# limix/CellRegMap

Hardware: AMD Instinct MI355X
Metric: variant-tests/sec (interaction test) (higher is better)
Workload: dtype f64

## Files before the change

cellregmap_amd/csrc/api_core.hip:

```cpp
#include <dlfcn.h>

#include <algorithm>
#include <atomic>
#include <cstdarg>
#include <mutex>

#include <map>

#include "crm_internal.h"
#include "eigh.h"

namespace crm {

static thread_local std::string g_error;

void set_error(const char* fmt, ...) {
    char buf[1024];
    va_list ap;
    va_start(ap, fmt);
    vsnprintf(buf, sizeof buf, fmt, ap);
    va_end(ap);
    g_error = buf;
}

// ... 216 lines not shown
    }
}

int crm_ctx_synchronize(crm_ctx* c) {
    return crm::guarded_on("crm_ctx_synchronize", c, [&]() -> int {
    if (!c) return CRM_ERR_ARG;
    CRM_HIP(hipSetDevice(c->device));
    CRM_HIP(hipStreamSynchronize(c->stream));
    return CRM_OK;
    });
}

int crm_set_block_variants(crm_ctx* c, int variants) {
    return crm::guarded_on("crm_set_block_variants", c, [&]() -> int {
    if (!c || variants < 0) return CRM_ERR_ARG;
    c->block_variants = variants == 0 ? 0 : (int)round_up(variants, 128);
    return CRM_OK;
    });
}

int crm_set_null_fit_polish(crm_ctx* c, int on) {
    return crm::guarded_on("crm_set_null_fit_polish", c, [&]() -> int {
    if (!c) return CRM_ERR_ARG;
    c->polish = on != 0;
    return CRM_OK;
    });
}

int crm_set_progress_callback(crm_ctx* c, void (*callback)(long, long, void*), void* user) {
    return crm::guarded_on("crm_set_progress_callback", c, [&]() -> int {
    if (!c) return CRM_ERR_ARG;
    if (callback) c->progress[std::this_thread::get_id()] = crm_ctx::Progress{callback, user};
    else c->progress.erase(std::this_thread::get_id());
    return CRM_OK;
    });
}

int crm_set_fast_rotation(crm_ctx* c, int on) {
    return crm::guarded_on("crm_set_fast_rotation", c, [&]() -> int {
    if (!c) return CRM_ERR_ARG;
    c->fast_T = on != 0;
    return CRM_OK;
    });
}

extern "C++" {
namespace crm {
namespace {
struct FormSlot { const char* name; int value; bool set; };
FormSlot g_forms[] = {{"gram_staged", 0, false}, {"kr_no_tail", 0, false}, {"nullfit_per_wave", 0, false}, {"kin_fold", 0, false},
                      {"eigh_one_stage", 0, false}, {"nullfit_exact", 0, false}, {"donor_pairs", 0, false},
                      {"pairs_without_kinship_term", 0, false}, {"flat_kappa_milli", 0, false}, {"chase_abort", 0, false}, {"nullfit_one_per_wave", 0, false},
                      {"kin_diag", 0, false}, {"donor_pairs_rotate", 0, false}, {"rho0_positions", 0, false},
                      {"rotation_tails", 0, false}};
std::mutex g_forms_mu;
}
int form(const char* name, int otherwise) {
    std::lock_guard<std::mutex> lock(g_forms_mu);
    for (const FormSlot& f : g_forms)
        if (strcmp(f.name, name) == 0) return f.set ? f.value : otherwise;
    return otherwise;
}
}
}

int crm_test_set_form(const char* name, int value, int reset) {
    return crm::guarded("crm_test_set_form", [&]() -> int {
    if (!name) return CRM_ERR_ARG;
    std::lock_guard<std::mutex> lock(crm::g_forms_mu);
    for (crm::FormSlot& f : crm::g_forms)
        if (strcmp(f.name, name) == 0) {
            f.value = value;
            f.set = reset == 0;
            return CRM_OK;
        }
    crm::set_error("crm_test_set_form: no kernel form is called '%s'", name);
    return CRM_ERR_ARG;
    });
}

int crm_kernel_timer_reset(crm_ctx* c) {
    return crm::guarded_on("crm_kernel_timer_reset", c, [&]() -> int {
    if (!c) return CRM_ERR_ARG;
    CRM_HIP(hipSetDevice(c->device));
    CRM_HIP(hipStreamSynchronize(c->stream));
    c->timed_used = 0;
    c->kr_flops = 0.0;
    c->timing = true;
    return CRM_OK;
    });
}

int crm_kernel_timer_stop(crm_ctx* c) {
    return crm::guarded_on("crm_kernel_timer_stop", c, [&]() -> int {
    if (!c) return CRM_ERR_ARG;
    c->timing = false;
    return CRM_OK;
    });
}

int crm_kernel_timer_read(crm_ctx* c, double* kr_ms, long* kr_launches, double* kr_flops,
                          double* total_ms) {
    return crm::guarded_on("crm_kernel_timer_read", c, [&]() -> int {
    if (!c) return CRM_ERR_ARG;
    CRM_HIP(hipSetDevice(c->device));
    CRM_HIP(hipStreamSynchronize(c->stream));
    double ms = 0.0;
// ... 250 lines not shown
```

cellregmap_amd/csrc/assemble.hip:

```cpp
#include <type_traits>

#include "nullfit.h"

namespace crm {

namespace {

constexpr int CH = 64;
constexpr int SLD = 66;

typedef double v4d __attribute__((ext_vector_type(4)));

template <int NTL, int NG = 1>
__global__ __launch_bounds__(256) void gram_ext_kernel(AssembleArgs a, double* __restrict__ Gext, int KT) {
    constexpr int ROWS = 16 * NTL, NTILES = NTL * (NTL + 1) / 2, NLOC = (NTILES + NG - 1) / NG, MAXT = (NLOC + 3) / 4,
                  RPT = ROWS / 4;
    extern __shared__ double Ss[];
    __shared__ int tile_ij[NTILES];
    __shared__ const double* tail_ptr[ROWS];
    const int b = blockIdx.x;
    const NullFitOut fit = a.fit[b];
    const AssembleRho R = a.rho[fit.rho_index];
    const int r = R.r;
    const double ratio = fit.v0 / fit.v1;
// ... 469 lines not shown
    }
    double* ME = wsm;
    double* Cm = ME + KT * k1;
    double* Z = Cm + k1 * k1;
    const long pos = a.sorted_pos[b];
    for (int e = tid; e < KT * k1; e += 256) {
        const int u = e / k1, f = e - u * k1;
        double plain;
        if (u < k0) plain = pos >= 0 ? a.wb_E1X[(long)f * a.wb_ldE1X + pos * k0 + u] : 0.0;
        else if (u < k0 + c) plain = a.wb_E1yW[(long)f * a.wb_ldE1yW + 1 + (u - k0)];
        else if (u == k0 + c) plain = a.wb_E1g[(long)f * a.wb_ldE1g + b];
        else plain = a.wb_E1yW[(long)f * a.wb_ldE1yW];
        ME[e] = (u < k0 && pos < 0) ? 0.0 : (plain - G[(long)u * KW + KT + f]) * inv;
    }
    for (int e = tid; e < k1 * k1; e += 256) {
        const int i = e / k1, j = e - i * k1;
        Cm[e] = (i == j ? 1.0 : 0.0) + g * (a.wb_EE[e] - G[(long)(KT + i) * KW + KT + j]) * inv;
    }
    __syncthreads();
    for (int j = 0; j < k1; j++) {
        if (tid == 0) Cm[j * k1 + j] = sqrt(Cm[j * k1 + j]);
        __syncthreads();
        const double l = Cm[j * k1 + j];
        for (int i = j + 1 + tid; i < k1; i += 256) Cm[i * k1 + j] /= l;
        __syncthreads();
        for (int e = tid; e < (k1 - j - 1) * (k1 - j - 1); e += 256) {
            const int i = j + 1 + e / (k1 - j - 1), q = j + 1 + e % (k1 - j - 1);
            if (q <= i) Cm[i * k1 + q] -= Cm[i * k1 + j] * Cm[q * k1 + j];
        }
        __syncthreads();
    }
    for (int u = tid; u < KT; u += 256) {
        for (int i = 0; i < k1; i++) {
            double s = ME[u * k1 + i];
            for (int q = 0; q < i; q++) s -= Cm[i * k1 + q] * Z[q * KT + u];
            Z[i * KT + u] = s / Cm[i * k1 + i];
        }
        for (int i = k1 - 1; i >= 0; i--) {
            double s = Z[i * KT + u];
            for (int q = i + 1; q < k1; q++) s -= Cm[q * k1 + i] * Z[q * KT + u];
            Z[i * KT + u] = s / Cm[i * k1 + i];
        }
    }
    __syncthreads();
    const double scale = fit.v1 * g;
    for (int e = tid; e < KT * KT; e += 256) {
        const int u = e / KT, v = e - u * KT;
        double s = 0.0;
        for (int f = 0; f < k1; f++) s += ME[u * k1 + f] * Z[f * KT + v];
        out[e] = G[(long)u * KW + v] + scale * s;
    }
}

constexpr int PMAX = CRM_MAX_COV_XWIDE + 1;

__global__ __launch_bounds__(128) void finalize_kernel(AssembleArgs a, const double* __restrict__ Gext,
                                                        int KT, double* __restrict__ rows) {
    extern __shared__ double fsm[];
    __shared__ int ok_flag, keep_flag;
    __shared__ double rescale;
    const int Pd = a.c + 1;
    double* Lm = fsm;
    double* xky = Lm + Pd * Pd;
    double* uvec = xky + Pd;
    double* vv = uvec + a.k0;
    double* ww = vv + Pd;
    double* dkxm = rows ? rows + (size_t)blockIdx.x * 2 * a.k0 * Pd : ww + Pd;
    double* solm = dkxm + a.k0 * Pd;
#define L(i, j) Lm[(i) * Pd + (j)]
#define dkx(j, i) dkxm[(j) * Pd + (i)]
#define sol(j, i) solm[(j) * Pd + (i)]
    const int b = blockIdx.x;
    const NullFitOut fit = a.fit[b];
    const int k0 = a.k0, c = a.c;
    const int P = c + 1;
    const double v1 = fit.v1;
    const double inv = 1.0 / v1;
    const double* __restrict__ Ge = Gext + (long)b * KT * KT;
    const int tid = threadIdx.x;
    auto plain_xx = [&](int i, int j) -> double {
        if (i > j) { int t = i; i = j; j = t; }
        if (j < c) return a.WW[i * c + j];
        if (i < c) return a.gW[(long)b * a.ld_gW + i];
        return a.gg[b];
    };
    auto plain_xy = [&](int i) -> double { return i < c ? a.Wy[i] : a.gy[b]; };

    if (tid == 0) {
        bool ok = true;
        for (int i = 0; i < P; i++) {
            for (int j = 0; j <= i; j++)
                L(i, j) = (plain_xx(i, j) - Ge[(long)(k0 + i) * KT + (k0 + j)]) * inv;
            xky[i] = (plain_xy(i) - Ge[(long)(k0 + i) * KT + (k0 + c + 1)]) * inv;
        }
        bool keep = true;
        for (int j = 0; j < P && ok; j++) {
            double d = L(j, j);
            for (int k = 0; k < j; k++) d -= L(j, k) * L(j, k);
            if (!(d > 0.0)) {
                if (j == c) keep = false;
                else ok = false;
                break;
            }
            const double l = sqrt(d);
            L(j, j) = l;
            for (int i = j + 1; i < P; i++) {
                double s = L(i, j);
                for (int k = 0; k < j; k++) s -= L(i, k) * L(j, k);
                L(i, j) = s / l;
            }
// ... 58 lines not shown
                for (int i = 0; i < used; i++) r -= xky[i] * xky[i];
                const double df = (double)a.n - (double)(c + (fit.use_g ? 1 : 0));
                rescale = 1.0 / fmax(r / df, 1.4901161193847656e-08);
            }
            for (int i = P - 1; i >= 0; i--) {
                double s = xky[i];
                for (int k = i + 1; k < P; k++) s -= L(k, i) * xky[k];
                xky[i] = s / L(i, i);
            }
        }
        ok_flag = ok ? 1 : 0;
    }
    __syncthreads();
    const bool ok = ok_flag != 0;
    const bool keep_g = keep_flag != 0;
    for (int j = tid; j < k0; j += blockDim.x) {
        double row[PMAX];
        for (int i = 0; i < P; i++) {
            double plain;
            if (i < c) plain = a.Z1[(long)b * a.ldZ1 + (long)(1 + i) * k0 + j];
            else plain = a.Z2[(long)b * a.ldZ2 + j];
            double v = (plain - Ge[(long)j * KT + (k0 + i)]) * inv;
            if (i == c && !keep_g) v = 0.0;
            row[i] = v;
            dkx(j, i) = v;
        }
        for (int i = 0; i < P; i++) {
            double s = row[i];
            for (int k = 0; k < i; k++) s -= L(i, k) * row[k];
            row[i] = s / L(i, i);
        }
        for (int i = P - 1; i >= 0; i--) {
            double s = row[i];
            for (int k = i + 1; k < P; k++) s -= L(k, i) * row[k];
            row[i] = s / L(i, i);
        }
        for (int i = 0; i < P; i++) sol(j, i) = row[i];
        const double dky = (a.Z1[(long)b * a.ldZ1 + j] - Ge[(long)j * KT + (k0 + c + 1)]) * inv;
        double u = dky;
        for (int i = 0; i < P; i++) u -= dkx(j, i) * xky[i];
        uvec[j] = u * rescale;
    }
    __syncthreads();
    if (tid == 0) {
        double q = 0.0;
        for (int j = 0; j < k0; j++) q += uvec[j] * uvec[j];
        a.Q[b] = ok ? 0.5 * q : NAN;
    }
    double* __restrict__ F = a.F + (long)b * k0 * k0;
    for (int e = tid; e < k0 * k0; e += blockDim.x) {
        const int j = e / k0, jp = e - j * k0;
        const int lo = j < jp ? j : jp, hi = j < jp ? jp : j;
        const long pidx = (long)lo * k0 - (long)lo * (lo - 1) / 2 + (hi - lo);
        double v = (a.Z3[(long)b * a.ldZ3 + pidx] - Ge[(long)j * KT + jp]) * inv;
        for (int i = 0; i < P; i++) v -= dkx(j, i) * sol(jp, i);
        F[e] = ok ? 0.5 * v * rescale : NAN;
    }
}
#undef L
#undef dkx
#undef sol

}

size_t woodbury_lds_bytes(int KT, int k1) { return sizeof(double) * ((size_t)2 * KT * k1 + (size_t)k1 * k1); }

size_t assemble_rows_scratch_doubles(int variants, int k0, int c) {
    const size_t P = (size_t)c + 1;
    const size_t lds = sizeof(double) * (P * P + 3 * P + k0 + 2 * (size_t)k0 * P);
    return lds > 150 * 1024 ? (size_t)variants * 2 * k0 * P : 0;
}

int launch_assemble(hipStream_t st, const AssembleArgs& a, int variants, double* Gext, double* fin_rows,
                    long* dma_launches) {
    if (variants <= 0) return CRM_OK;
    const int KT0 = a.k0 + a.c + 2;
    const int KT = KT0 + (a.wb_k1 > 0 ? a.wb_k1 : 0);
    double* const Gfin = Gext;
    if (a.wb_k1 > 0) {
        if (KT > CRM_MAX_GRAM_ROWS || woodbury_lds_bytes(KT0, a.wb_k1) > 150 * 1024 || !a.wb_Gw) {
            set_error("assemble: unrelated-donor form with %d + %d rows outside its supported range", KT0, a.wb_k1);
            return CRM_ERR_INTERNAL;
        }
        Gext = a.wb_Gw;
    }
    const int P = a.c + 1;
    const size_t fin_small = sizeof(double) * ((size_t)P * P + 3 * P + a.k0);
    size_t fin_lds = fin_small + sizeof(double) * 2 * (size_t)a.k0 * P;
    const bool rows_global = fin_lds > 150 * 1024;
    if (rows_global) fin_lds = fin_small;
    if (a.k0 > CRM_MAX_K0 || a.c > CRM_MAX_COV_XWIDE || KT > CRM_MAX_GRAM_ROWS || (rows_global && !fin_rows)) {
        set_error("assemble: k0=%d, c=%d outside the supported range (k0 <= %d, c <= %d, k0 + c + 2 <= %d)", a.k0, a.c,
                  CRM_MAX_K0, CRM_MAX_COV_XWIDE, CRM_MAX_GRAM_ROWS);
        return CRM_ERR_UNSUPPORTED;
    }
    const int ts = (KT + 15) / 16;
    bool dma = ts <= 9 && a.ldA % 2 == 0 && (reinterpret_cast<uintptr_t>(a.A) & 15) == 0 && !form("gram_staged", 0);
    for (int i = 0; dma && i < CRM_MAX_RHO; i++) {
        const AssembleRho& R = a.rho[i];
        if (R.r <= 0 && !R.ty) continue;
        dma = R.ldW % 2 == 0 && R.ldT % 2 == 0 && ((reinterpret_cast<uintptr_t>(R.ty) | reinterpret_cast<uintptr_t>(R.tW) |
                                                    reinterpret_cast<uintptr_t>(R.T)) & 15) == 0;
    }
    if (a.wb_k1 > 0) dma = dma && a.wb_ldR % 2 == 0 && (reinterpret_cast<uintptr_t>(a.wb_R) & 15) == 0;
#define CRM_GRAM_DMA(KERNEL, LDS_DOUBLES, NTL)                                                                \
    do {                                                                                                      \
        const size_t lds = sizeof(double) * LDS_DOUBLES(NTL);                                                 \
        if (lds > 60 * 1024)                                                                                  \
            CRM_HIP(hipFuncSetAttribute(reinterpret_cast<const void*>(&KERNEL<NTL>),                          \
                                        hipFuncAttributeMaxDynamicSharedMemorySize, (int)lds));               \
        hipLaunchKernelGGL(KERNEL<NTL>, dim3(variants), dim3(256), lds, st, a, Gext, KT);                     \
    } while (0)
#define CRM_GRAM_DMA_WIDE(NTL) CRM_GRAM_DMA(gram_ext_dma_wide_kernel, gram_dma_wide_lds_doubles, NTL)
    if (dma) {
        if (ts <= 2) CRM_GRAM_DMA(gram_ext_dma_kernel, gram_dma_lds_doubles, 2);
        else if (ts <= 4) CRM_GRAM_DMA(gram_ext_dma_kernel, gram_dma_lds_doubles, 4);
        else if (ts == 5) CRM_GRAM_DMA_WIDE(5);
        else if (ts == 6) CRM_GRAM_DMA_WIDE(6);
        else if (ts == 7) CRM_GRAM_DMA_WIDE(7);
        else if (ts == 8) CRM_GRAM_DMA_WIDE(8);
        else CRM_GRAM_DMA_WIDE(9);
    }
#undef CRM_GRAM_DMA_WIDE
#undef CRM_GRAM_DMA
#define CRM_GRAM(NTL)                                                                                         \
    do {                                                                                                      \
        const size_t lds = sizeof(double) * 16 * NTL * SLD;                                                   \
        if (lds > 60 * 1024)                                                                                  \
            CRM_HIP(hipFuncSetAttribute(reinterpret_cast<const void*>(&gram_ext_kernel<NTL>),                 \
                                        hipFuncAttributeMaxDynamicSharedMemorySize, (int)lds));               \
        hipLaunchKernelGGL(gram_ext_kernel<NTL>, dim3(variants), dim3(256), lds, st, a, Gext, KT);            \
    } while (0)
#define CRM_GRAM_GROUPS(NTL, NG)                                                                              \
    do {                                                                                                      \
        const size_t lds = sizeof(double) * 16 * NTL * SLD;                                                   \
        CRM_HIP(hipFuncSetAttribute(reinterpret_cast<const void*>(&gram_ext_kernel<NTL, NG>),                 \
                                    hipFuncAttributeMaxDynamicSharedMemorySize, (int)lds));                   \
        hipLaunchKernelGGL((gram_ext_kernel<NTL, NG>), dim3(variants, NG), dim3(256), lds, st, a, Gext, KT);  \
    } while (0)
    if (dma) {
    } else if (ts <= 2) CRM_GRAM(2);
    else if (ts <= 4) CRM_GRAM(4);
    else if (ts <= 6) CRM_GRAM(6);
    else if (ts <= 7) CRM_GRAM(7);
    else if (ts <= 9) CRM_GRAM(9);
    else if (ts <= 12) CRM_GRAM_GROUPS(12, 2);
    else if (ts <= 15) CRM_GRAM_GROUPS(15, 4);
    else CRM_GRAM_GROUPS(18, 4);
#undef CRM_GRAM
#undef CRM_GRAM_GROUPS
    CRM_HIP(hipGetLastError());
    if (dma && dma_launches) ++*dma_launches;
    if (a.wb_k1 > 0) {
        const size_t lds = woodbury_lds_bytes(KT0, a.wb_k1);
        if (lds > 60 * 1024)
            CRM_HIP(hipFuncSetAttribute(reinterpret_cast<const void*>(&woodbury_kernel),
                                        hipFuncAttributeMaxDynamicSharedMemorySize, (int)lds));
        hipLaunchKernelGGL(woodbury_kernel, dim3(variants), dim3(256), lds, st, a, a.wb_Gw, KT0, Gfin);
        CRM_HIP(hipGetLastError());
    }
    if (fin_lds > 60 * 1024)
        CRM_HIP(hipFuncSetAttribute(reinterpret_cast<const void*>(&finalize_kernel),
                                    hipFuncAttributeMaxDynamicSharedMemorySize, (int)fin_lds));
    hipLaunchKernelGGL(finalize_kernel, dim3(variants), dim3(128), fin_lds, st, a, Gfin, KT0, rows_global ? fin_rows : nullptr);
    CRM_HIP(hipGetLastError());
    return CRM_OK;
}

}
```

cellregmap_amd/csrc/scan.hip:

```cpp
#include <algorithm>

#include "nullfit.h"
#include "objects.h"

using namespace crm;

namespace crm {

static int ctx_cus(const crm_ctx* ctx) {
    int cus = 256;
    if (hipDeviceGetAttribute(&cus, hipDeviceAttributeMultiprocessorCount, ctx->device) != hipSuccess || cus < 1) cus = 256;
    return cus;
}

constexpr double COLLINEAR_TAU = 1e-2;

__global__ void flat_probe_fit_kernel(const crm::NullFitOut* __restrict__ fit, int count, double sign,
                                      crm::NullFitOut* __restrict__ out) {
    const int b = blockIdx.x * blockDim.x + threadIdx.x;
    if (b >= count) return;
    crm::NullFitOut f = fit[b];
    const double tiny = 2.220446049250313e-16;
    const double d = fmin(fmax(f.delta, tiny), 1.0 - tiny);
    const double x = log(d) - log1p(-d);
// ... 11 lines not shown
    const int b = blockIdx.y;
    const int j = blockIdx.x * blockDim.x + threadIdx.x;
    if (b >= nb || j >= cols) return;
    const int ri = fit[b].rho_index;
    if (ri < 0) return;
    double* slab = T + ((size_t)ri * blk + b) * ldT;
    if (restore) slab[j] = rows[(size_t)b * ldT + j];
    else rows[(size_t)b * ldT + j] = slab[j];
}

constexpr double STOP_SHIFT_C = 2.5e-13;
constexpr double FLAT_KAPPA = 1.0;
constexpr double RHO_KAPPA = 1.0;
constexpr int FLAT_REC = 10;

struct ScanOut {
    double *pv, *rho1, *e2, *g2, *eps2, *Q, *lml, *delta, *scale, *lambda, *F;
    int* ifault = nullptr;
    double* liu = nullptr;
    int* flags = nullptr;
    double* bound_Q = nullptr;
    double* bound_p = nullptr;
    bool exact = false;
    double* logp = nullptr;
    int* status = nullptr;
};

static bool scan_slow_forms(const crm_gene* g0) {
    return g0->k0 + g0->c + 2 > 144 || g0->k0 > 128 || assemble_rows_scratch_doubles(1, g0->k0, g0->c) > 0;
}
static int scan_block_variants(const crm_ctx* ctx, const crm_gene* g0, long count) {
    long auto_blk = (long)(16.0 * (1ull << 30) / (sizeof(double) * (double)g0->k0 * (double)g0->bg->ldq)) / 128 * 128;
    auto_blk = std::max<long>(256, std::min<long>(auto_blk, CRM_MAX_AUTO_BLOCK));
    int BLK = (int)std::min<long>(ctx->block_variants > 0 ? ctx->block_variants : auto_blk, round_up(count, 128));
    if (g0->c > CRM_MAX_COV_WIDE) BLK = std::min(BLK, 512);
    if (scan_slow_forms(g0)) BLK = std::min(BLK, 512);
    return BLK;
}

enum class Route {
    collapsed,
    direct,
    kin_unfolded,
    kin_folded,
    unrelated,
};

constexpr int SLOT_ONE = 0, SLOT_RHO = 1, SLOT_KIN = 2 * CRM_MAX_RHO + 4;

struct ScanPlan {
    Route route = Route::direct;
    bool fastT = false, slow_forms = false, skip_pairs = true, cross = false;
    bool e1_pairs = false, e1_sym = false, donor_pairs = false, wb_rotate = false, pairs_unfolded = false;
    int ng = 1, BLK = 0, pair_cap = 0;
    long ldb = 0, ldp = 0, ldA = 0, ldAw = 0, ldT = 0, ldZ1 = 0, ldZ2 = 0, ldZ3 = 0, ld_ah = 0, ld_xg = 0, ldP = 0, ldPd = 0,
         pd_slab = 0, ldwb = 0, ld_gW = 0, th_slab = 0, s_rows = 0;
    size_t s_bytes = 0;
    int ks1 = 1, ks2 = 1, ks3 = 1, ks_h = 1, fold_split6 = 1, fold_split3 = 1, donor_pair_splits = 1;
    int npair = 0, KT = 0, KK = 0, kin_probs = 0;
    long kdim = 0, mp = 0, xrows = 0;
    bool collapsed() const { return route == Route::collapsed; }
    bool kin() const { return route == Route::kin_unfolded || route == Route::kin_folded || route == Route::unrelated; }
    bool folded() const { return route == Route::kin_folded || route == Route::unrelated; }
    bool wb() const { return route == Route::unrelated; }
    bool through_H() const { return fastT && (ng > 1 || kin()); }
    int z1_slot() const { return SLOT_KIN + kin_probs; }
};

static double largest_rank(const crm_background* bg) {
    double rbar = 1.0;
    for (int i = 0; i < bg->nrho; i++) rbar = std::max(rbar, (double)bg->r[i]);
    return rbar;
}

static ScanPlan plan_scan(const std::vector<crm_gene*>& genes, const crm_panel* panel, const int* idx_G, bool allow_collapse,
                          long count) {
    const crm_gene* g0 = genes[0];
    const crm_background* bg = g0->bg;
    const crm_ctx* ctx = bg->ctx;
    const int ng = (int)genes.size(), nrho = bg->nrho, c = g0->c, k0 = g0->k0;
    const long n = bg->n, np = bg->n_pad, ldq = bg->ldq;
    ScanPlan P;
    P.ng = ng;
    P.slow_forms = scan_slow_forms(g0);
    const int BLK = P.BLK = scan_block_variants(ctx, g0, count);
    P.pair_cap = BLK;
    if (ng > 1) {
        const char* cap_env = getenv("CRM_PAIR_BUFFER_GB");
        const double cap_gb = cap_env && atof(cap_env) > 0 ? atof(cap_env) : 128.0;
        const double per_pair = 2.0 * sizeof(double) * k0 * (double)ldq;
        const long most = (long)std::min(nrho, ng) * BLK, least = (long)std::min(nrho, ng) * std::min(BLK, 128);
        P.pair_cap = (int)std::max<long>(least, std::min<long>(most, (long)(cap_gb * (1ull << 30) / per_pair)));
    }
    const int max_pairs = P.pair_cap;
    P.ldb = BLK + 128;
    P.ldp = max_pairs + 128;
    P.ldA = P.ldT = ldq;
    P.npair = k0 * (k0 + 1) / 2;
    P.ldZ1 = round_up((long)k0 * (1 + c), 128), P.ldZ2 = round_up(k0, 128), P.ldZ3 = round_up(P.npair, 128);
    P.KT = k0 + c + 2;
    P.ld_gW = round_up(std::max(c, CRM_MAX_COV), 8);
    const int mt_blk = (BLK + GEMM_BM - 1) / GEMM_BM;
    P.ks1 = split_for(np, (long)mt_blk * (P.ldZ1 / GEMM_BN) * ng);
    P.ks2 = split_for(np, (long)mt_blk * (P.ldZ2 / GEMM_BN));
    P.ks3 = split_for(np, (long)mt_blk * (P.ldZ3 / GEMM_BN));
    P.th_slab = std::max<long>(bg->ldh, bg->kin && bg->kin_fold ? bg->kin_kdim + (bg->kin_wb ? GEMM_BK : 0) : 0) * P.ldb;
// ... 17 lines not shown
    bool kin_pays = false;
    if (bg->kin) {
        const double rbar = largest_rank(bg);
        const double kk = fold ? (double)bg->kin_kdim : (double)bg->ldh;
        const double prep = fold ? 2.0 * bg->kin_rows * bg->kin_k2 + 2.0 * (double)np * bg->kin_k1
                                 : 2.0 * bg->kin_rows * P.KK + 2.0 * (double)bg->kin_groups_pad * bg->kin_cols * bg->kin_k2;
        kin_pays = prep + 2.0 * kk * rbar < 0.9 * 2.0 * (double)n * rbar || ctx->kin_route >= 2;
    }
    const bool kin_route = bg->kin && P.fastT && ctx->kin_route > 0 && kin_pays && !(ng > 1 && ctx->tune.shared_h >= 0) &&
                           P.s_bytes <= ((size_t)48 << 30);
    const bool kfold = kin_route && fold;
    const int wb_k1 = bg->kin ? bg->kin_k1 : 0;
    bool wb = false;
    constexpr int WB_MAX_ROWS = 144;
    if (kfold && bg->kin_wb && !P.slow_forms && c + 1 <= 128 && P.KT + wb_k1 <= WB_MAX_ROWS &&
        woodbury_lds_bytes(P.KT, wb_k1) <= 150 * 1024) {
        wb = (double)bg->kin_kdim * largest_rank(bg) * k0 > 8.0 * (P.KT + wb_k1) * (P.KT + wb_k1) * (double)bg->wb_P ||
             form("kin_diag", 1) >= 2;
    }
    P.route = collapsed ? Route::collapsed : wb ? Route::unrelated : kfold ? Route::kin_folded
            : kin_route ? Route::kin_unfolded : Route::direct;
    P.ldAw = wb ? std::max<long>(P.ldA, bg->wb_ldp) : P.ldA;
    P.ldwb = wb ? bg->wb_ldp : 0;
    P.kdim = kfold ? bg->kin_kdim : bg->ldh;
    P.ldP = round_up((long)(bg->kin ? bg->kin_k1 : 0) * k0, 128);
    P.e1_pairs = kfold && sizeof(double) * (double)np * (double)P.ldP <= 8.0 * (1ull << 30);
    if (kfold) {
        const long tiles6 = P.e1_pairs ? ((long)BLK + GEMM_BM - 1) / GEMM_BM * (P.ldP / 128) : ((long)BLK * k0 + GEMM_BM - 1) / GEMM_BM;
        const long slots6 = P.e1_pairs || bg->kin_k1 > 64 ? 512 : 768;
        double best = 0.0;
        for (int sps = 1; sps <= 8 && np / GEMM_BK / sps >= 64; sps++) {
            const double rounds = (double)(tiles6 * sps) / (double)slots6, eff = rounds / std::ceil(rounds);
            if (eff > best + 0.02) { best = eff; P.fold_split6 = sps; }
        }
        const long tiles3 = (long)((bg->kin_k1 + GEMM_BM - 1) / GEMM_BM) * ((BLK + 127) / 128);
        while (tiles3 * P.fold_split3 < 1024 && P.fold_split3 < 16 && np / GEMM_BK / (P.fold_split3 + 1) >= 16) P.fold_split3++;
    }
    P.e1_sym = P.e1_pairs && bg->kin_k1 == k0;
    P.ldPd = round_up((long)P.npair, 128);
    P.pd_slab = (std::max<long>(BLK, max_pairs) + 128) * P.ldPd;
    if (P.e1_sym && bg->kin_k2 == k0 && donor_pairs_serves(k0) && form("donor_pairs", 1)) {
        const double peak = 78.6e12, hbm = 4.0e12;
        const double t_kr = 2.0 * bg->kin_rows * (double)k0 * k0 / (0.6 * peak) + 2.0 * (double)np * P.npair / (0.92 * peak);
        const double t_pairs = 2.0 * bg->kin_rows * (double)P.npair / (0.8 * peak) +
                               (double)bg->kin_groups * (2.0 * P.npair + (double)k0 * k0) * sizeof(double) / hbm;
        const bool fits = sizeof(double) * (double)bg->kin_groups * (double)P.pd_slab <= 8.0 * (1ull << 30);
        P.donor_pairs = fits && (t_pairs < t_kr || form("donor_pairs", 1) >= 2);
        const long wgs = (std::max<long>(BLK, 1) + 3) / 4;
        while ((wgs * P.donor_pair_splits) % 768 != 0 && wgs * P.donor_pair_splits < 4 * 768 && P.donor_pair_splits < 8 &&
               P.donor_pair_splits < bg->kin_groups)
            P.donor_pair_splits++;
    }
    P.wb_rotate = wb && P.donor_pairs && donor_pairs_rotate_serves(k0) && form("donor_pairs_rotate", 1) != 0;
    if (kin_route && !kfold && bg->kin_k1 == k0 && bg->kin_k2 == k0 && donor_pairs_serves(k0) && form("donor_pairs", 1) &&
        bg->kin_cols + 1 <= bg->kin_ldh) {
        const double cost_kr = 2.0 * bg->kin_rows * (double)P.KK * k0 + 2.0 * (double)bg->kin_groups_pad * bg->kin_cols * bg->kin_k2 * k0;
        const double cost_pairs = 2.0 * bg->kin_rows * (double)P.npair + 2.0 * (double)(bg->kin_cols + 1) * bg->kin_groups_pad * (double)P.ldPd;
        const bool fits = sizeof(double) * (double)bg->kin_groups_pad * (double)P.pd_slab <= 8.0 * (1ull << 30) &&
                          sizeof(double) * (double)(bg->kin_cols + 1) * (double)P.pd_slab <= (double)P.s_bytes;
        P.pairs_unfolded = fits && (cost_pairs < 0.8 * cost_kr || form("donor_pairs", 1) >= 2);
    }
    P.skip_pairs = form("pairs_without_kinship_term", 1) != 0;
    P.kin_probs = bg->kin ? bg->kin_groups * (bg->kin_wb ? 2 : 1) + bg->kin_k2 + 16 : 0;
    return P;
}

static long donor_run_records(const crm_background* bg, const GemmProblem& p, long c_step, GemmProblem* out) {
    long maxlen = GEMM_BK;
    for (long d = 0; d < bg->kin_groups; d++) {
        const long r0 = bg->kin_row0[d];
        GemmProblem q = p;
        q.X = p.X + r0 * p.ldx;
        if (p.E) q.E = p.E + r0 * p.lde;
        q.Y = p.Y + r0 * p.ldy; q.C = p.C + d * c_step; q.cells = bg->kin_len[d];
        maxlen = std::max(maxlen, bg->kin_len[d]);
        out[d] = q;
    }
    return maxlen;
}

static void woodbury_records(const crm_background* bg, const GemmProblem& p, long x_step, GemmProblem* out) {
    for (long d = 0; d < bg->kin_groups; d++) {
        GemmProblem q = p;
        q.X = p.X + d * x_step; q.Y = bg->wb_U.as<double>() + (size_t)d * bg->wb_k2pad * 128; q.ldy = 128;
        q.C = p.C + d * bg->kin_k2; q.N = bg->kin_k2; q.cells = bg->wb_k2pad;
        out[d] = q;
    }
}

struct SameColumns { const double* A; long lda; const double* B; long ldb; long rows; };
static int same_columns(hipStream_t st, int* d_flag, int k, std::initializer_list<SameColumns> pairs, bool& same) {
    int h_flag = 0;
    CRM_HIP(hipMemsetAsync(d_flag, 0, sizeof(int), st));
    for (const SameColumns& q : pairs) CRM_TRY(launch_same_columns(st, q.A, q.lda, q.B, q.ldb, q.rows, k, d_flag));
    CRM_HIP(hipMemcpyAsync(&h_flag, d_flag, sizeof(int), hipMemcpyDeviceToHost, st));
    CRM_HIP(hipStreamSynchronize(st));
    same = h_flag == 0;
    return CRM_OK;
}

struct Block {
    long done = 0, col0 = 0;
    int nb = 0;
    double* Gb = nullptr;
    double* Gt = nullptr;
    double* Gx = nullptr;
// ... 722 lines not shown
    SubRange sub_range(const Block& B, int b0) const {
        SubRange R;
        R.b0 = b0;
        R.nb = B.nb - b0;
        R.done = B.done + b0;
        if (ng > 1) {
            long pairs = 0;
            int take = 0;
            for (; b0 + take < B.nb; take++) {
                unsigned seen = 0;
                for (int gi = 0; gi < ng; gi++) {
                    const NullFitOut& f = h_fit[(size_t)gi * P.BLK + b0 + take];
                    if (!no_kinship_term(f)) seen |= 1u << f.rho_index;
                }
                const int here = __builtin_popcount(seen);
                if (take > 0 && pairs + here > P.pair_cap) break;
                pairs += here;
            }
            R.nb = take;
        }
        return R;
    }

    int select_pairs(const Block& B, const SubRange& R, Pairs& Q) {
        const int nb = R.nb, BLK = P.BLK;
        const NullFitOut* fit = h_fit.data() + R.b0;
        std::fill(pair_of.begin(), pair_of.end(), -1);
        long with_pair = 0;
        for (int gi = 0; gi < ng; gi++)
            for (int b = 0; b < nb; b++) {
                const NullFitOut& f = fit[(size_t)gi * BLK + b];
                if (no_kinship_term(f)) continue;
                pair_of[(size_t)f.rho_index * BLK + b] = 0;
                with_pair++;
            }
        ctx->tests_without_pair += (long)ng * nb - with_pair;
        if (with_pair == 0) pair_of[(size_t)fit[0].rho_index * BLK] = 0;
        for (int i = 0; i < nrho; i++) {
            Q.start[i] = Q.npairs;
            for (int b = 0; b < nb; b++) {
                if (pair_of[(size_t)i * BLK + b] == 0) {
                    pair_of[(size_t)i * BLK + b] = Q.npairs;
                    h_ord[Q.npairs++] = b;
                }
            }
            Q.cnt[i] = Q.npairs - Q.start[i];
        }
        Q.start[nrho] = Q.npairs;
        for (int gi = 0; gi < ng; gi++)
            for (int b = 0; b < nb; b++) {
                const NullFitOut& f = fit[(size_t)gi * BLK + b];
                h_pos[(size_t)gi * BLK + b] = no_kinship_term(f) ? -1 : pair_of[(size_t)f.rho_index * BLK + b];
            }
        CRM_HIP(hipMemcpyAsync(d_pos, h_pos.data(), sizeof(int) * (size_t)BLK * ng, hipMemcpyHostToDevice, st));
        if (P.wb() && ng > 1) {
            std::vector<int> h_posw((size_t)BLK * ng, -1);
            for (int gi = 0; gi < ng; gi++)
                for (int b = 0; b < nb; b++)
                    if (h_pos[(size_t)gi * BLK + b] >= 0) h_posw[(size_t)gi * BLK + b] = b;
            CRM_HIP(hipMemcpyAsync(d_posw, h_posw.data(), sizeof(int) * h_posw.size(), hipMemcpyHostToDevice, st));
            CRM_HIP(hipStreamSynchronize(st));
        }
        CRM_HIP(hipMemcpyAsync(d_ord, h_ord.data(), sizeof(int) * Q.npairs, hipMemcpyHostToDevice, st));
        return launch_gather_block(st, B.Gt + R.b0, P.ldb, P.xrows, P.xrows, nullptr, d_ord, Q.npairs, ctx->ws_Gs.as<double>(),
                                   P.ldp, (int)P.ldp);
    }

    int direct_splits(const Pairs& Q, AGroups& A, bool* tail_of) {
        A.a_slab = (size_t)P.pair_cap * k0 * P.ldA;
        long row_tiles = 0;
        int mn = 1;
        for (int i = 0; i < nrho; i++)
            if (Q.cnt[i] > 0) { row_tiles += ((long)Q.cnt[i] * k0 + GEMM_BM - 1) / GEMM_BM; mn = std::max(mn, bg->r[i]); }
        const int cap = (int)std::min<size_t>(8, ((size_t)16 << 30) / std::max<size_t>(sizeof(double) * A.a_slab, 1));
        A.kr_split = kr_split_for(ctx, row_tiles, mn, 1, np, std::max(cap, 1));
        if (A.kr_split > 1) CRM_TRY(ctx->ws_A.ensure(sizeof(double) * A.a_slab * A.kr_split));
        if (A.kr_split > 1 || !ctx->tune.glds || ctx->tune.bn == 64 || ctx->tune.bn == 160 || form("kr_no_tail", 0)) return CRM_OK;
        long tail_row_tiles = 0, main_tiles = 0;
        for (int i = 0; i < nrho; i++) {
            if (Q.cnt[i] == 0) continue;
            const int N = bg->r[i], rem = N % 128;
            const long rt = ((long)Q.cnt[i] * k0 + GEMM_BM - 1) / GEMM_BM;
            main_tiles += rt * ((N + 127) / 128);
            if (N >= 1024 && rem > 0 && rem <= 32) {
                tail_of[i] = true;
                tail_row_tiles += rt;
                A.tail_maxn = std::max(A.tail_maxn, 128 + rem);
            }
        }
        if (tail_row_tiles == 0 || main_tiles <= 1024) {
            std::fill(tail_of, tail_of + CRM_MAX_RHO, false);
        } else {
            const int saved_bn = ctx->tune.bn;
            ctx->tune.bn = 160;
            A.tail_split = kr_split_for(ctx, tail_row_tiles, A.tail_maxn, 1, np, std::max(cap, 1));
            ctx->tune.bn = saved_bn;
            if (A.tail_split > 1) CRM_TRY(ctx->ws_A.ensure(sizeof(double) * A.a_slab * A.tail_split));
        }
        return CRM_OK;
    }

    void a_records(const Pairs& Q, bool via_H, const bool* tail_of, AGroups& A) {
        const double kin_rows = P.folded() ? bg->kin_k1 + bg->kin_groups * (long)bg->kin_k2 : bg->cols;
        for (int i = 0; i < nrho; i++) {
            if (Q.cnt[i] == 0 || P.wb()) continue;
            GemmProblem p{};
            p.X = ctx->ws_Gs.as<double>() + Q.start[i]; p.ldx = P.ldp;
            p.C = ctx->ws_A.as<double>() + (size_t)Q.start[i] * k0 * P.ldA;
            if (P.collapsed()) {
                p.Y = tab->Bd.as<double>() + (size_t)i * P.mp * k0 * ldq; p.ldy = (long)k0 * ldq; p.ldc = (long)k0 * P.ldA;
                p.M = Q.cnt[i]; p.N = (int)((long)k0 * ldq);
            } else if (via_H) {
                if (P.kin() && ng == 1) {
                    p.X = (P.folded() ? ctx->ws_S.as<double>() : ctx->ws_AH.as<double>()) + (size_t)Q.start[i] * k0; p.ldx = P.ld_ah;
                } else {
                    p.X = ctx->ws_XG.as<double>() + (size_t)Q.start[i] * k0; p.ldx = P.ld_xg;
                }
                p.Y = P.folded() ? bg->MixK[i].as<double>() : bg->Mix[i].as<double>(); p.ldy = ldq; p.ldc = P.ldA;
                p.M = Q.cnt[i] * k0; p.N = bg->r[i] > 0 ? bg->r[i] : 1;
                A.kr_flops += 2.0 * kin_rows * (double)bg->r[i] * (double)k0 * (double)Q.cnt[i];
            } else {
                p.E = d_Ep; p.lde = g0->ld_ep; p.k0 = k0; p.Y = bg->Q0[i].as<double>(); p.ldy = ldq; p.ldc = P.ldA;
                p.M = Q.cnt[i] * k0; p.N = bg->r[i] > 0 ? bg->r[i] : 1;
                A.kr_flops += 2.0 * (double)n * (double)bg->r[i] * (double)k0 * (double)Q.cnt[i];
                if (tail_of[i]) {
                    GemmProblem t = p;
                    const int rem = 128 + p.N % 128;
                    p.N -= rem;
                    t.Y = p.Y + p.N; t.C = p.C + p.N; t.N = rem;
                    A.tails.push_back(t);
                }
            }
            if (P.kin() && p.N >= 1024 && p.N % 128 > 0 && p.N % 128 <= 16 && p.ldx % 2 == 0 &&
                (reinterpret_cast<uintptr_t>(p.X) & 15) == 0 && !form("kr_no_tail", 0)) {
                GemmProblem t = p;
                const int rem = p.N % 128;
                A.kr_flops -= 2.0 * kin_rows * (double)rem * (double)k0 * (double)Q.cnt[i];
                p.N -= rem;
                t.Y = p.Y + p.N; t.C = p.C + p.N; t.N = rem;
                A.spectrum_tails.push_back(t);
            }
            A.max_m = std::max(A.max_m, p.M);
            A.max_n = std::max(A.max_n, p.N);
            probs[A.nz++] = p;
        }
    }

    struct DonorCols { bool in_pair_order; const double* G; long ldg; int ncol; };
    int donor_columns(const Block& B, const SubRange& R, const Pairs& Q, DonorCols& D) {
        D.in_pair_order = ng == 1;
        D.G = D.in_pair_order ? ctx->ws_Gs.as<double>() : B.Gt + R.b0;
        D.ldg = D.in_pair_order ? P.ldp : P.ldb;
        D.ncol = D.in_pair_order ? Q.npairs : R.nb;
        const int blk_cols = (int)(P.ldb - R.b0);
        return launch_gather_rows(st, D.G, D.ldg, bg->kin_map.as<int>(), bg->kin_rows, D.in_pair_order ? (int)D.ldg : blk_cols,
                                  ctx->ws_Gk.as<double>(), D.ldg);
    }
    int gather_pairs(const double* src, long rows, const Pairs& Q) {
        const int xg_cols = (int)std::min<long>(P.ld_xg, round_up((long)Q.npairs * k0, 128) + 128);
        return launch_gather_slabs(st, src, P.ld_ah, rows, d_ord, Q.npairs, k0, ctx->ws_XG.as<double>(), P.ld_xg, xg_cols);
    }

    int folded_S(const Block& B, const SubRange& R, const Pairs& Q) {
        DonorCols D;
        CRM_TRY(donor_columns(B, R, Q, D));
        double* S = ctx->ws_S.as<double>();
        double* Gk = ctx->ws_Gk.as<double>();
        const int k1 = bg->kin_k1, k2 = bg->kin_k2, ncol = D.ncol, npair = P.npair;
        const long groups = bg->kin_groups, ld_ah = P.ld_ah;
        std::vector<GemmProblem> kp((size_t)groups + P.fold_split6);
        GemmProblem p{};
        p.X = Gk; p.ldx = D.ldg;
        if (P.donor_pairs) {
            p.Y = g0->kinEE.as<double>(); p.ldy = g0->ld_ee; p.C = ctx->ws_Pd.as<double>(); p.ldc = P.ldPd;
            p.M = ncol; p.N = npair;
        } else if (k2 == 1) {
            p.Y = g0->kinUE.as<double>(); p.ldy = g0->ld_ep; p.C = S + (size_t)k1 * ld_ah; p.ldc = k0; p.M = ncol; p.N = k0;
        } else {
            p.E = g0->kinEp.as<double>(); p.lde = g0->ld_ep; p.k0 = k0; p.Y = bg->kin_Y.as<double>(); p.ldy = bg->kin_ldy;
            p.C = S + (size_t)k1 * ld_ah; p.ldc = ld_ah; p.M = ncol * k0; p.N = k2;
        }
        const long maxlen = donor_run_records(bg, p, P.donor_pairs ? P.pd_slab : (long)k2 * ld_ah, kp.data());
        const long stages_all = np / GEMM_BK, per = (stages_all + P.fold_split6 - 1) / P.fold_split6;
        const long e1_slab = (long)k1 * ld_ah;
        int slices = 0;
        long chunk_max = GEMM_BK;
        if (P.e1_pairs) {
            GemmProblem& e = kp[groups];
            e.X = D.G; e.ldx = D.ldg; e.Y = g0->kinP.as<double>(); e.ldy = P.ldP;
            e.C = ctx->ws_AH.as<double>(); e.ldc = P.ldP; e.M = ncol; e.N = k1 * k0;
            if (P.e1_sym) { e.Y = d_EE; e.ldy = g0->ld_ee; e.N = npair; }
        }
        for (int sps = 0; sps < P.fold_split6 && !P.e1_pairs; sps++) {
            const long s0 = sps * per, s1 = std::min(stages_all, s0 + per);
            if (s1 <= s0) break;
            GemmProblem& e = kp[groups + slices++];
            e.X = D.G + s0 * GEMM_BK * D.ldg; e.ldx = D.ldg;
            e.E = d_Ep + s0 * GEMM_BK * g0->ld_ep; e.lde = g0->ld_ep; e.k0 = k0;
            e.Y = bg->H.as<double>() + s0 * GEMM_BK * bg->ldh; e.ldy = bg->ldh;
            e.C = ctx->ws_AH.as<double>() + (size_t)sps * e1_slab; e.ldc = ld_ah;
            e.M = ncol * k0; e.N = k1; e.cells = (s1 - s0) * GEMM_BK;
            chunk_max = std::max(chunk_max, e.cells);
        }
// ... 40 lines not shown
        const int k1 = bg->kin_k1, k2 = bg->kin_k2, ncol = D.ncol, npair = P.npair;
        const long groups = bg->kin_groups, mk = bg->kin_cols, KK = P.KK, ld_ah = P.ld_ah;
        GemmProblem p{};
        p.X = ctx->ws_Gk.as<double>(); p.ldx = D.ldg;
        if (P.pairs_unfolded) {
            double* Pd = ctx->ws_Pd.as<double>();
            double* Z = S;
            std::vector<GemmProblem> kp((size_t)groups + 1);
            p.Y = g0->kinEE.as<double>(); p.ldy = g0->ld_ee; p.C = Pd; p.ldc = P.ldPd; p.M = ncol; p.N = npair;
            const long maxlen = donor_run_records(bg, p, P.pd_slab, kp.data());
            GemmProblem& z = kp[groups];
            z.X = bg->kin_hKd.as<double>(); z.ldx = bg->kin_ldh;
            z.Y = Pd; z.ldy = P.pd_slab; z.C = Z; z.ldc = P.pd_slab; z.M = (int)mk + 1; z.N = (int)((long)ncol * P.ldPd);
            return with_records(SLOT_KIN, kp, [&](GemmProblem* d_kp) -> int {
                CRM_TRY(launch_gemm_tn(ctx, d_kp, (int)groups, ncol, npair, maxlen, false, 0, 1, 0));
                CRM_TRY(launch_gemm_tn(ctx, d_kp + groups, 1, (int)mk + 1, (int)((long)ncol * P.ldPd), bg->kin_groups_pad, false, 0, 1, 0));
                CRM_TRY(launch_donor_pairs_expand(st, Z, P.pd_slab, P.ldPd, (int)mk, ncol, k0, k1, AH, ld_ah, Pd, P.pd_slab, 1, 1, mk));
                CRM_TRY(launch_pair_rows_sym(st, Z + (size_t)mk * P.pd_slab, P.ldPd, ncol, k0, AH, ld_ah));
                ctx->donor_pair_blocks++;
                if (!D.in_pair_order) CRM_TRY(gather_pairs(AH, bg->ldh, Q));
                return CRM_OK;
            });
        }
        std::vector<GemmProblem> kp((size_t)groups + k2);
        p.E = g0->kinEp.as<double>(); p.lde = g0->ld_ep; p.k0 = k0; p.Y = bg->kin_Y.as<double>(); p.ldy = bg->kin_ldy;
        p.C = S; p.ldc = ld_ah; p.M = ncol * k0; p.N = (int)KK;
        const long maxlen = donor_run_records(bg, p, KK * ld_ah, kp.data());
        for (int j = 0; j < k2; j++) {
            GemmProblem& q = kp[groups + j];
            q.X = bg->kin_hKd.as<double>(); q.ldx = bg->kin_ldh; q.Y = S + (size_t)j * ld_ah; q.ldy = KK * ld_ah;
            q.C = AH + (size_t)(k1 + (long)j * mk) * ld_ah; q.ldc = ld_ah; q.M = (int)mk; q.N = ncol * k0;
        }
        return with_records(SLOT_KIN, kp, [&](GemmProblem* d_kp) -> int {
            CRM_TRY(launch_kr_transposed(ctx, d_kp, (int)groups, ncol * k0, (int)KK, maxlen, k0));
            CRM_TRY(launch_gemm_tn(ctx, d_kp + groups, k2, (int)mk, ncol * k0, bg->kin_groups_pad, false, 0, 1, 0));
            CRM_TRY(launch_kin_sum_e1(st, S, ld_ah, (int)KK, k2, k1, (int)groups, (long)ncol * k0, AH, ld_ah));
            if (!D.in_pair_order) CRM_TRY(gather_pairs(AH, bg->ldh, Q));
            return CRM_OK;
        });
    }

    int direct_AH(const Block& B, const SubRange& R, const Pairs& Q, AGroups& A) {
        GemmProblem p{};
        p.X = B.Gt + R.b0; p.ldx = P.ldb; p.E = d_Ep; p.lde = g0->ld_ep; p.k0 = k0; p.Y = bg->H.as<double>(); p.ldy = bg->ldh;
        p.C = ctx->ws_AH.as<double>(); p.ldc = P.ld_ah; p.M = R.nb * k0; p.N = (int)bg->cols;
        CRM_TRY(upload(SLOT_ONE, &p, 1));
        CRM_TRY(launch_kr_transposed(ctx, d_probs + SLOT_ONE, 1, p.M, p.N, np, k0));
        A.kr_flops += 2.0 * (double)n * (double)bg->cols * (double)k0 * (double)R.nb;
        return gather_pairs(ctx->ws_AH.as<double>(), bg->ldh, Q);
    }

    int woodbury_S(const SubRange& R, const Pairs& Q) {
        const long groups = bg->kin_groups;
        const int ncol = ng == 1 ? Q.npairs : R.nb;
        std::vector<GemmProblem> kp((size_t)groups);
        GemmProblem p{};
        p.X = ctx->ws_S.as<double>() + (size_t)bg->kin_k1 * P.ld_ah; p.ldx = P.ld_ah;
        p.C = ctx->ws_A.as<double>(); p.ldc = P.ldAw; p.M = ncol * k0;
        woodbury_records(bg, p, (long)bg->kin_k2 * P.ld_ah, kp.data());
        return with_records(SLOT_KIN, kp, [&](GemmProblem* d_kp) {
            return launch_gemm_tn(ctx, d_kp, (int)groups, ncol * k0, bg->kin_k2, bg->wb_k2pad, false, 0, 1, 0);
        });
    }

    int form_A(const Block& B, const SubRange& R, const Pairs& Q) {
        bool via_H = P.kin();
        if (P.fastT && ng > 1 && !P.kin()) {
            double direct = 0.0, via = (double)R.nb * (double)bg->cols * (double)n;
            for (int i = 0; i < nrho; i++) {
                direct += (double)Q.cnt[i] * bg->r[i] * (double)n;
                via += (double)Q.cnt[i] * bg->r[i] * (double)bg->ldh;
            }
            via_H = ctx->tune.shared_h < 0 ? via < 0.9 * direct : ctx->tune.shared_h > 0;
        }
        const bool direct = !P.collapsed() && !via_H;
        if (direct)
            for (int i = 0; i < nrho; i++)
                if (Q.cnt[i] > 0) CRM_TRY(crm_background_require_q0(bg, i));
        AGroups A;
        bool tail_of[CRM_MAX_RHO] = {false};
        if (direct) CRM_TRY(direct_splits(Q, A, tail_of));
        a_records(Q, via_H, tail_of, A);
        const bool timing = !P.wb() && ctx->timing && ctx->timed_used < 65536;
        if (timing) CRM_TRY(timer_open(!P.kin()));
        if (P.folded()) CRM_TRY(folded_S(B, R, Q));
        else if (P.kin()) CRM_TRY(unfolded_AH(B, R, Q));
        else if (via_H) CRM_TRY(direct_AH(B, R, Q, A));
        CRM_TRY(upload(SLOT_ONE, probs.data(), A.nz));
        GemmProblem* d_A = d_probs + SLOT_ONE;
        if (P.collapsed()) {
            CRM_TRY(launch_gemm_tn(ctx, d_A, A.nz, A.max_m, (int)((long)k0 * ldq), P.mp, false, 0, 1, 0));
        } else if (P.wb()) {
            if (!P.wb_rotate) CRM_TRY(woodbury_S(R, Q));
        } else if (P.kin()) {
            if (timing) CRM_HIP(hipEventRecord(ctx->timed[ctx->timed_used].first, st));
            struct Restore { crm_ctx* c; ~Restore() { c->tune.tag = 0; } } restore{ctx};
            ctx->tune.tag = 1;
            CRM_TRY(launch_gemm_tn(ctx, d_A, A.nz, A.max_m, A.max_n, P.kdim, false, 0, 1, 0));
        } else if (via_H) {
            CRM_TRY(launch_gemm_tn(ctx, d_A, A.nz, A.max_m, A.max_n, P.kdim, false, 0, 1, 0));
        } else {
            CRM_TRY(launch_gemm_tn(ctx, d_A, A.nz, A.max_m, A.max_n, np, true, k0, A.kr_split, (long)A.a_slab));
            CRM_TRY(launch_reduce_splits(st, ctx->ws_A.as<double>(), (long)Q.npairs * k0 * P.ldA, A.kr_split, (long)A.a_slab));
            if (!A.tails.empty()) {
                const int saved_bn = ctx->tune.bn;
                ctx->tune.bn = 160;
                struct Restore { crm_ctx* c; int bn; ~Restore() { c->tune.bn = bn; } } restore{ctx, saved_bn};
// ... 554 lines not shown
```

Measured before the change: 73720.

## Add Cholesky-based Y^T Y Woodbury kernel and block-order donor columns

Adds a Woodbury kernel that Cholesky-factors the small capacitance matrix in LDS, applies the triangular solve to the stacked right-hand side, and forms the correction as a symmetric Y^T Y product with FP64 MFMA over upper-triangular 16x16 tiles. Results are mirrored, and finalize gets a flag to read only the computed triangle. Separately, the Woodbury path now keeps donor columns in block order rather than pair order, which skips a gather and turns positions into identity indices. Both are on by default and change several interacting stages, with some risk of numerical or indexing differences.

```diff
diff --git a/cellregmap_amd/csrc/api_core.hip b/cellregmap_amd/csrc/api_core.hip
--- a/cellregmap_amd/csrc/api_core.hip
+++ b/cellregmap_amd/csrc/api_core.hip
@@ -292,7 +292,8 @@
                       {"eigh_one_stage", 0, false}, {"nullfit_exact", 0, false}, {"donor_pairs", 0, false},
                       {"pairs_without_kinship_term", 0, false}, {"flat_kappa_milli", 0, false}, {"chase_abort", 0, false}, {"nullfit_one_per_wave", 0, false},
                       {"kin_diag", 0, false}, {"donor_pairs_rotate", 0, false}, {"rho0_positions", 0, false},
-                      {"rotation_tails", 0, false}};
+                      {"rotation_tails", 0, false}, {"woodbury_ytY", 0, false},
+                      {"wb_block_order", 0, false}};
 std::mutex g_forms_mu;
 }
 int form(const char* name, int otherwise) {
diff --git a/cellregmap_amd/csrc/assemble.hip b/cellregmap_amd/csrc/assemble.hip
--- a/cellregmap_amd/csrc/assemble.hip
+++ b/cellregmap_amd/csrc/assemble.hip
@@ -545,10 +545,100 @@
     }
 }
 
+__global__ __launch_bounds__(256) void woodbury_yty_kernel(AssembleArgs a, const double* __restrict__ Gw, int KT,
+                                                           double* __restrict__ Gext) {
+    extern __shared__ double wsm[];
+    const int k1 = a.wb_k1, KW = KT + k1, k0 = a.k0, c = a.c;
+    const int NR = k1 + KT, LD = NR | 1;
+    const int b = blockIdx.x, tid = threadIdx.x;
+    const int lane = tid & 63, wave = __builtin_amdgcn_readfirstlane(tid >> 6);
+    const NullFitOut fit = a.fit[b];
+    const double g = fit.v0 * a.rho[fit.rho_index].rho;
+    const double inv = 1.0 / fit.v1;
+    const double* __restrict__ G = Gw + (long)b * KW * KW;
+    double* __restrict__ out = Gext + (long)b * KT * KT;
+    if (!(g > 0.0)) {
+        for (int e = tid; e < KT * KT; e += 256) out[e] = G[(long)(e / KT) * KW + e % KT];
+        return;
+    }
+    double* AT = wsm;
+    const long pos = a.sorted_pos[b];
+    for (int e = tid; e < KT * k1; e += 256) {
+        const int u = e / k1, f = e - u * k1;
+        double plain;
+        if (u < k0) plain = pos >= 0 ? a.wb_E1X[(long)f * a.wb_ldE1X + pos * k0 + u] : 0.0;
+        else if (u < k0 + c) plain = a.wb_E1yW[(long)f * a.wb_ldE1yW + 1 + (u - k0)];
+        else if (u == k0 + c) plain = a.wb_E1g[(long)f * a.wb_ldE1g + b];
+        else plain = a.wb_E1yW[(long)f * a.wb_ldE1yW];
+        AT[f * LD + k1 + u] = (u < k0 && pos < 0) ? 0.0 : (plain - G[(long)u * KW + KT + f]) * inv;
+    }
+    for (int e = tid; e < k1 * k1; e += 256) {
+        const int i = e / k1, j = e - i * k1;
+        if (j <= i) AT[j * LD + i] = (i == j ? 1.0 : 0.0) + g * (a.wb_EE[e] - G[(long)(KT + i) * KW + KT + j]) * inv;
+    }
+    __syncthreads();
+    if (wave == 0) {
+        const double l = sqrt(AT[0]);
+        for (int R = lane; R < NR; R += 64) AT[R] = R == 0 ? l : AT[R] / l;
+    }
+    __syncthreads();
+    for (int j = 0; j + 1 < k1; j++) {
+        const double* colj = AT + j * LD;
+        const double lnext = wave == 0 ? sqrt(fma(-colj[j + 1], colj[j + 1], AT[(j + 1) * LD + j + 1])) : 0.0;
+        for (int R = ((j + 1) & ~63) + lane; R < NR; R += 64) {
+            const double aR = R > j ? colj[R] : 0.0;
+            for (int q0 = j + 1 + wave; q0 < k1; q0 += 16) {
+                double lq[4], cv[4];
+#pragma unroll
+                for (int m = 0; m < 4; m++) {
+                    const int q = q0 + 4 * m;
+                    const bool on = q < k1 && R >= q;
+                    lq[m] = on ? colj[q] : 0.0;
+                    cv[m] = on ? AT[q * LD + R] : 0.0;
+                }
+#pragma unroll
+                for (int m = 0; m < 4; m++) {
+                    const int q = q0 + 4 * m;
+                    if (!(q < k1 && R >= q)) continue;
+                    double v = fma(-aR, lq[m], cv[m]);
+                    if (q == j + 1) v = R == q ? lnext : v / lnext;
+                    AT[q * LD + R] = v;
+                }
+            }
+        }
+        __syncthreads();
+    }
+    const int ts = (KT + 15) / 16, l15 = lane & 15, l4 = lane >> 4;
+    const double scale = fit.v1 * g;
+    const double* __restrict__ Y = AT + k1;
+    int t = 0;
+    for (int ti = 0; ti < ts; ti++)
+        for (int tj = ti; tj < ts; tj++, t++) {
+            if ((t & 3) != wave) continue;
+            const int u = 16 * ti + l15, v = 16 * tj + l15;
+            v4d acc = (v4d){0.0, 0.0, 0.0, 0.0};
+            for (int f0 = 0; f0 < k1; f0 += 4) {
+                const int f = f0 + l4;
+                const double fa = (f < k1 && u < KT) ? Y[f * LD + u] : 0.0;
+                const double fb = (f < k1 && v < KT) ? Y[f * LD + v] : 0.0;
+                acc = __builtin_amdgcn_mfma_f64_16x16x4f64(fa, fb, acc, 0, 0, 0);
+            }
+#pragma unroll
+            for (int reg = 0; reg < 4; reg++) {
+                const int row = 16 * ti + l4 + 4 * reg;
+                if (row < KT && v < KT && v >= row) {
+                    const double s = scale * acc[reg];
+                    out[(long)row * KT + v] = G[(long)row * KW + v] + s;
+                    if (v != row) out[(long)v * KT + row] = G[(long)v * KW + row] + s;
+                }
+            }
+        }
+}
+
 constexpr int PMAX = CRM_MAX_COV_XWIDE + 1;
 
 __global__ __launch_bounds__(128) void finalize_kernel(AssembleArgs a, const double* __restrict__ Gext,
-                                                        int KT, double* __restrict__ rows) {
+                                                        int KT, double* __restrict__ rows, int sym) {
     extern __shared__ double fsm[];
     __shared__ int ok_flag, keep_flag;
     __shared__ double rescale;
@@ -713,8 +803,9 @@
         const int j = e / k0, jp = e - j * k0;
         const int lo = j < jp ? j : jp, hi = j < jp ? jp : j;
         const long pidx = (long)lo * k0 - (long)lo * (lo - 1) / 2 + (hi - lo);
-        double v = (a.Z3[(long)b * a.ldZ3 + pidx] - Ge[(long)j * KT + jp]) * inv;
-        for (int i = 0; i < P; i++) v -= dkx(j, i) * sol(jp, i);
+        const int ja = sym ? lo : j, jb = sym ? hi : jp;
+        double v = (a.Z3[(long)b * a.ldZ3 + pidx] - Ge[(long)ja * KT + jb]) * inv;
+        for (int i = 0; i < P; i++) v -= dkx(ja, i) * sol(jb, i);
         F[e] = ok ? 0.5 * v * rescale : NAN;
     }
 }
@@ -812,18 +903,20 @@
 #undef CRM_GRAM_GROUPS
     CRM_HIP(hipGetLastError());
     if (dma && dma_launches) ++*dma_launches;
+    const bool yty = a.wb_k1 > 0 && form("woodbury_ytY", 1) != 0;
     if (a.wb_k1 > 0) {
-        const size_t lds = woodbury_lds_bytes(KT0, a.wb_k1);
-        if (lds > 60 * 1024)
-            CRM_HIP(hipFuncSetAttribute(reinterpret_cast<const void*>(&woodbury_kernel),
-                                        hipFuncAttributeMaxDynamicSharedMemorySize, (int)lds));
-        hipLaunchKernelGGL(woodbury_kernel, dim3(variants), dim3(256), lds, st, a, a.wb_Gw, KT0, Gfin);
+        const size_t lds = yty ? sizeof(double) * a.wb_k1 * (size_t)((KT0 + a.wb_k1) | 1) : woodbury_lds_bytes(KT0, a.wb_k1);
+        const void* fn = yty ? reinterpret_cast<const void*>(&woodbury_yty_kernel) : reinterpret_cast<const void*>(&woodbury_kernel);
+        if (lds > 60 * 1024) CRM_HIP(hipFuncSetAttribute(fn, hipFuncAttributeMaxDynamicSharedMemorySize, (int)lds));
+        if (yty) hipLaunchKernelGGL(woodbury_yty_kernel, dim3(variants), dim3(256), lds, st, a, a.wb_Gw, KT0, Gfin);
+        else hipLaunchKernelGGL(woodbury_kernel, dim3(variants), dim3(256), lds, st, a, a.wb_Gw, KT0, Gfin);
         CRM_HIP(hipGetLastError());
     }
     if (fin_lds > 60 * 1024)
         CRM_HIP(hipFuncSetAttribute(reinterpret_cast<const void*>(&finalize_kernel),
                                     hipFuncAttributeMaxDynamicSharedMemorySize, (int)fin_lds));
-    hipLaunchKernelGGL(finalize_kernel, dim3(variants), dim3(128), fin_lds, st, a, Gfin, KT0, rows_global ? fin_rows : nullptr);
+    hipLaunchKernelGGL(finalize_kernel, dim3(variants), dim3(128), fin_lds, st, a, Gfin, KT0, rows_global ? fin_rows : nullptr,
+                       yty ? 1 : 0);
     CRM_HIP(hipGetLastError());
     return CRM_OK;
 }
diff --git a/cellregmap_amd/csrc/scan.hip b/cellregmap_amd/csrc/scan.hip
--- a/cellregmap_amd/csrc/scan.hip
+++ b/cellregmap_amd/csrc/scan.hip
@@ -87,6 +87,7 @@
     Route route = Route::direct;
     bool fastT = false, slow_forms = false, skip_pairs = true, cross = false;
     bool e1_pairs = false, e1_sym = false, donor_pairs = false, wb_rotate = false, pairs_unfolded = false;
+    bool wb_block = false;
     int ng = 1, BLK = 0, pair_cap = 0;
     long ldb = 0, ldp = 0, ldA = 0, ldAw = 0, ldT = 0, ldZ1 = 0, ldZ2 = 0, ldZ3 = 0, ld_ah = 0, ld_xg = 0, ldP = 0, ldPd = 0,
          pd_slab = 0, ldwb = 0, ld_gW = 0, th_slab = 0, s_rows = 0;
@@ -210,6 +211,7 @@
             P.donor_pair_splits++;
     }
     P.wb_rotate = wb && P.donor_pairs && donor_pairs_rotate_serves(k0) && form("donor_pairs_rotate", 1) != 0;
+    P.wb_block = wb && (ng > 1 || form("wb_block_order", 1) != 0);
     if (kin_route && !kfold && bg->kin_k1 == k0 && bg->kin_k2 == k0 && donor_pairs_serves(k0) && form("donor_pairs", 1) &&
         bg->kin_cols + 1 <= bg->kin_ldh) {
         const double cost_kr = 2.0 * bg->kin_rows * (double)P.KK * k0 + 2.0 * (double)bg->kin_groups_pad * bg->kin_cols * bg->kin_k2 * k0;
@@ -1038,6 +1040,12 @@
                 const NullFitOut& f = fit[(size_t)gi * BLK + b];
                 h_pos[(size_t)gi * BLK + b] = no_kinship_term(f) ? -1 : pair_of[(size_t)f.rho_index * BLK + b];
             }
+        if (P.wb_block && ng == 1) {
+            for (int b = 0; b < nb; b++)
+                if (h_pos[b] >= 0) h_pos[b] = b;
+            CRM_HIP(hipMemcpyAsync(d_pos, h_pos.data(), sizeof(int) * (size_t)BLK, hipMemcpyHostToDevice, st));
+            return CRM_OK;
+        }
         CRM_HIP(hipMemcpyAsync(d_pos, h_pos.data(), sizeof(int) * (size_t)BLK * ng, hipMemcpyHostToDevice, st));
         if (P.wb() && ng > 1) {
             std::vector<int> h_posw((size_t)BLK * ng, -1);
@@ -1134,7 +1142,7 @@
 
     struct DonorCols { bool in_pair_order; const double* G; long ldg; int ncol; };
     int donor_columns(const Block& B, const SubRange& R, const Pairs& Q, DonorCols& D) {
-        D.in_pair_order = ng == 1;
+        D.in_pair_order = ng == 1 && !P.wb_block;
         D.G = D.in_pair_order ? ctx->ws_Gs.as<double>() : B.Gt + R.b0;
         D.ldg = D.in_pair_order ? P.ldp : P.ldb;
         D.ncol = D.in_pair_order ? Q.npairs : R.nb;
@@ -1281,7 +1289,7 @@
 
     int woodbury_S(const SubRange& R, const Pairs& Q) {
         const long groups = bg->kin_groups;
-        const int ncol = ng == 1 ? Q.npairs : R.nb;
+        const int ncol = P.wb_block ? R.nb : Q.npairs;
         std::vector<GemmProblem> kp((size_t)groups);
         GemmProblem p{};
         p.X = ctx->ws_S.as<double>() + (size_t)bg->kin_k1 * P.ld_ah; p.ldx = P.ld_ah;
```

After: 75120 (median of 6 runs). 1.02x the previous value.
